# PriviligedLearningDistributedAerial/imitation

Measured on AMD Instinct MI355X. Metric: env-steps/sec (whole node) + final eval return, GAIL HalfCheetah-v4 at 1/2/4/8 MI355X, higher is better.
Workload: dtype mixed (fp32 master weights and accumulation; PPO products as split-bf16 x3 ~fp32, discriminator bf16); 1 GPU; model=GAIL: FeedForward32Policy[32,32]+RunningNorm / BasicRewardNet(32,32)+RunningNorm, global_batch=4096, seq_len=512, parallelism=dp1, engine=device, env=HalfCheetah-v4

## Files before the change

### csrc/kernels/ppo_rc_kernel.h

```cpp
#pragma once
#include <hip/hip_runtime.h>
#include <stdlib.h>

#include "ia/engine.h"
#include "ia/wave.h"
#include "launchers.h"


namespace ia {
namespace rc {


typedef float f4 __attribute__((ext_vector_type(4)));
typedef __bf16 bf16;
typedef __bf16 bf16x8 __attribute__((ext_vector_type(8)));
typedef __attribute__((address_space(3))) bf16 lbf;
typedef __attribute__((address_space(3))) bf16x8 lbf8;
typedef __attribute__((address_space(3))) float lf;
typedef __attribute__((address_space(3))) f4 lf4;

constexpr int kL = kWaveMaxLayers;

__device__ __forceinline__ f4 mfma(float a, float b, f4 c) { return __builtin_amdgcn_mfma_f32_16x16x4f32(a, b, c, 0, 0, 0); }
__device__ __forceinline__ int rfl(int v) { return __builtin_amdgcn_readfirstlane(v); }
// ... 199 lines not shown
}
__device__ __forceinline__ void img_store1(lf* L, int off, int rp, int f, int row, float v) {
  lch* p = (lch*)L + 4 * off + (f >> 4) * img_strip(rp) + img_unit(row, (f >> 2) & 3) + 2 * (f & 3);
  const bf16 h = (bf16)v;
  *(lbf*)p = h;
  *(lbf*)(p + img_lo(rp)) = (bf16)(v - (float)h);
}
__device__ __forceinline__ bf16x8 img_read8(const lch* a0, const lch* a1) {
  const bf16x4 x = __builtin_amdgcn_ds_read_tr16_b64_v4bf16((lbf4*)a0);
  const bf16x4 y = __builtin_amdgcn_ds_read_tr16_b64_v4bf16((lbf4*)a1);
  return cat4(x, y);
}

__device__ __forceinline__ f4 mfma_bf16(bf16x8 a, bf16x8 b, f4 c) { return __builtin_amdgcn_mfma_f32_16x16x32_bf16(a, b, c, 0, 0, 0); }

template <int N>
__device__ __forceinline__ void dw_tiles(const lf* L, const int* izo, const int* iho, int d1, int lo, int ksteps, f4* acc) {
  const lch* Lb = (const lch*)L;
  constexpr int GS = N >= 12 ? 2 : 4;
#pragma unroll
  for (int i0 = 0; i0 < N; i0 += GS) {
    for (int ks = 0; ks < ksteps; ++ks) {
      bf16x8 zh[GS], zl[GS], hh[GS], hl[GS];
#pragma unroll
      for (int i = 0; i < GS; ++i) {
        if (i0 + i >= N) continue;
        const lch* zp = Lb + izo[i0 + i] + kImgKStep * ks;
        const lch* hp = Lb + iho[i0 + i] + kImgKStep * ks;
        zh[i] = img_read8(zp, zp + d1);
        zl[i] = img_read8(zp + lo, zp + lo + d1);
        hh[i] = img_read8(hp, hp + d1);
        hl[i] = img_read8(hp + lo, hp + lo + d1);
      }
#pragma unroll
      for (int i = 0; i < GS; ++i) {
        if (i0 + i >= N) continue;
        acc[i0 + i] = mfma_bf16(zh[i], hh[i], acc[i0 + i]);
        acc[i0 + i] = mfma_bf16(zh[i], hl[i], acc[i0 + i]);
        acc[i0 + i] = mfma_bf16(zl[i], hh[i], acc[i0 + i]);
      }
    }
  }
}

__host__ __device__ __forceinline__ int bf3_ld(int k) { return k + 8; }
__device__ __forceinline__ int bf3_pos_in0(int f) { return 8 * (f & 3) + (f >> 2); }
__device__ __forceinline__ int bf3_pos_h(int f) { return 32 * (f >> 5) + 8 * ((f >> 2) & 3) + 4 * ((f >> 4) & 1) + (f & 3); }

__device__ __forceinline__ void split8(const float (&v)[8], bf16x8& hi, bf16x8& lo) {
#pragma unroll
  for (int j = 0; j < 8; ++j) {
    const bf16 h = (bf16)v[j];
    hi[j] = h;
    lo[j] = (bf16)(v[j] - (float)h);
  }
}

__device__ __forceinline__ f4 bf3_tile(const lbf* a, int lo_off, bf16x8 bh, bf16x8 bl, f4 acc) {
  const bf16x8 ah = *(const lbf8*)a;
  const bf16x8 al = *(const lbf8*)(a + lo_off);
  acc = mfma_bf16(ah, bh, acc);
  acc = mfma_bf16(ah, bl, acc);
  return mfma_bf16(al, bh, acc);
}

__device__ __forceinline__ f4 bf3_mm(bf16x8 ah, bf16x8 al, bf16x8 bh, bf16x8 bl, f4 acc) {
  acc = mfma_bf16(ah, bh, acc);
  acc = mfma_bf16(ah, bl, acc);
  return mfma_bf16(al, bh, acc);
}

template <int KT>
__device__ __forceinline__ void bf3_store_w(lf* L, const PPORcGeo& g, int q, int l, int o, int i, float v, int nl) {
  const bf16 h = (bf16)v;
  const bf16 lo = (bf16)(v - (float)h);
  const int kin = l == 0 ? 32 : 16 * KT;
  const int rows = (g.dout[q][l] + 15) & ~15;
  lbf* wf = (lbf*)(L + g.wf_off[q][l]) + o * bf3_ld(kin) + (l == 0 ? bf3_pos_in0(i) : bf3_pos_h(i));
  wf[0] = h;
  wf[rows * bf3_ld(kin)] = lo;
  if (l > 0) {
    const int kout = l == nl - 1 ? 32 : 16 * KT;
    const int trows = (g.din[q][l] + 15) & ~15;
    lbf* wt = (lbf*)(L + g.wt_off[q][l]) + i * bf3_ld(kout) + bf3_pos_h(o);
    wt[0] = h;
    wt[trows * bf3_ld(kout)] = lo;
  }
}

template <int KT>
__device__ __forceinline__ void bf3_store_tile(lf* L, int kind, int wf, int wfl, int wt, int wtl, int r16, int kk,
                                               const float (&v)[4]) {
  typedef __bf16 bf16x4 __attribute__((ext_vector_type(4)));
  typedef __attribute__((address_space(3))) bf16x4 lbf4;
  bf16x4 h4, l4;
#pragma unroll
  for (int j = 0; j < 4; ++j) {
    const bf16 h = (bf16)v[j];
    h4[j] = h;
    l4[j] = (bf16)(v[j] - (float)h);
  }
  lbf* Lb = (lbf*)L;
  const int ldi = kind == 0 ? bf3_ld(32) : bf3_ld(16 * KT);
  lbf* pf = Lb + wf + 4 * kk * ldi + (kind == 0 ? 8 * (r16 & 3) + (r16 >> 2) : 8 * (r16 >> 2) + (r16 & 3));
#pragma unroll
  for (int j = 0; j < 4; ++j) {
    pf[j * ldi] = h4[j];
    pf[j * ldi + wfl] = l4[j];
  }
  if (kind != 0) {
    const int ldo = kind == 2 ? bf3_ld(32) : bf3_ld(16 * KT);
    lbf* pt = Lb + wt + r16 * ldo + 8 * kk;
    *(lbf4*)pt = h4;
    *(lbf4*)(pt + wtl) = l4;
  }
}

constexpr bool rc_is_bf3(int KT, int S0T, int NLT, int HWT, int CWT, int NW) {
  return HWT == 16 * KT && NLT == 3 && S0T != 0 && (S0T > 0 ? S0T : -S0T) <= 8 && CWT == 64 && (NW == 4 || KT == 2);
}

template <int KT, int KW, int KB, int S0T, int NLT, int ACTT, int HWT, int CWT, int DT, int NW, int LEAN = 0>
__global__ __launch_bounds__(64 * NW) void ppo_rc_kernel(PPOArgs a, PPORcGeo g) {
  constexpr int KI = KW + KB;
  constexpr bool kLean = LEAN != 0;
  unsigned long long* const prof = kLean ? nullptr : a.prof;
  constexpr int kThreads = 64 * NW;
  constexpr int kWaves = NW;
  constexpr int kHalf = NW / 2;
  extern __shared__ __attribute__((aligned(16))) float lds_raw[];
  lf* L = (lf*)lds_raw;
  const int tid = threadIdx.x;
  const int w = rfl(tid >> 6), lane = tid & 63;
  const int r16 = lane & 15, kk = lane >> 4;
  const bool ns = g.ns != 0;
  int bid = (int)blockIdx.x;
  if (g.xcd > 1) {
    if (bid % g.xcd) return;
    bid /= g.xcd;
  }
  const int q = ns ? (bid & 1) : w / kHalf;
  const int gw = ns ? w : w % kHalf;
  const int grp = ns ? (bid >> 1) : bid;
  const int G = kLean ? 1 : g.G, nch = g.nch, cw = CWT > 0 ? CWT : g.cw;
  const int CH = G * nch;
  const int Bg = CH * cw;
  const int RT = cw / 16;
  const bool rows_wave = gw < RT;
  const int nl = NLT > 0 ? NLT : (q == 0 ? a.n_pi : a.n_vf);
  const int D = a.D, A = a.A;
  constexpr int S0M = S0T > 0 ? S0T : (S0T < 0 ? -S0T : 16);
  const int s0 = S0T > 0 ? S0T : (D + 3) / 4;
  constexpr bool BF3 = rc_is_bf3(KT, S0T, NLT, HWT, CWT, NW);
  const bool gauss = DT >= 0 ? DT == 0 : !a.discrete;
  const bool has_ls = gauss && a.log_std_off >= 0;
  float am[4];
#pragma unroll
  for (int j = 0; j < 4; ++j) am[j] = 4 * (lane >> 4) + j < a.A ? 1.f : 0.f;
  const int n_mb = a.rows / Bg;
  const int K = a.n_epochs * n_mb;
  const float invB = 1.f / (float)Bg;
  const float c_half_log2pi = 0.91893853320467274f;
  const int n_items = rfl(g.n_items);

  for (int i = tid; i < g.lds_floats; i += kThreads) L[i] = 0.f;
  __syncthreads();
#pragma unroll
  for (int qq = 0; qq < 2; ++qq) {
#pragma unroll
    for (int l = 0; l < kL; ++l) {
      if (l >= (qq == 0 ? a.n_pi : a.n_vf) || (ns && qq != q)) continue;
      const LG y = lg(g, qq, l);
      const int wo = qq == 0 ? a.pi_w_off[l] : a.vf_w_off[l];
      const int bo = qq == 0 ? a.pi_b_off[l] : a.vf_b_off[l];
      for (int i = tid; i < y.dout * y.din; i += kThreads) {
        const int o = i / y.din, c = i - o * y.din;
        if constexpr (BF3) bf3_store_w<KT>(L, g, qq, l, o, c, a.params[wo + i], qq == 0 ? a.n_pi : a.n_vf);
        else L[y.w + o * y.ldw + c] = a.params[wo + i];
      }
      for (int i = tid; i < y.dout; i += kThreads) L[y.b + i] = a.params[bo + i];
    }
  }
  if (tid < 16) L[g.ls_off + tid] = (has_ls && tid < A && !(ns && q != 0)) ? a.params[a.log_std_off + tid] : 0.f;
  const int nc = tid - (kThreads - 64);
  const bool norm_lane = a.has_norm && nc >= 0 && nc < D;
  float run_m = 0.f, run_v = 1.f, run_c = 0.f;
  if (norm_lane) {
    run_m = a.norm_mean[nc];
    run_v = a.norm_var[nc];
    run_c = a.norm_count_i ? (float)a.norm_count_i[0] : a.norm_count[0];
  }
  const int n_witems = rfl(g.n_witems);
  const int wb = ns ? rfl(g.wbase[q]) : 0, nwq = ns ? rfl(g.nwit[q]) : n_witems;
  const int bb = ns ? rfl(g.bbase[q]) : n_witems, nbq = ns ? rfl(g.nbit[q]) : n_items - n_witems;
  float gm[KW][4], gv[KW][4];
  f4 gg[KW];
  float wmst[BF3 ? KW : 1][4];
  float bm[KB], bv[KB], bg[KB];
#pragma unroll
  for (int it = 0; it < KW; ++it) {
#pragma unroll
    for (int j = 0; j < 4; ++j) gm[it][j] = gv[it][j] = 0.f;
    gg[it] = {0.f, 0.f, 0.f, 0.f};
    if (w + it * kWaves < nwq) {
      const int desc = rfl(g.items[wb + w + it * kWaves]);
      const int iq = desc & 1, il = (desc >> 1) & 3, ta = (desc >> 5) & 15, tb = (desc >> 9) & 15;
      const int din = g.din[iq][il], dout = g.dout[iq][il];
      const int wo = iq == 0 ? a.pi_w_off[il] : a.vf_w_off[il];
      const int in = 16 * tb + r16;
#pragma unroll
      for (int j = 0; j < 4; ++j) {
        const int o = 16 * ta + 4 * kk + j;
        if constexpr (BF3) wmst[it][j] = 0.f;
        if (o < dout && in < din) {
          gm[it][j] = a.exp_avg[wo + o * din + in];
          gv[it][j] = a.exp_avg_sq[wo + o * din + in];
          if constexpr (BF3) wmst[it][j] = a.params[wo + o * din + in];
        }
      }
    }
  }
#pragma unroll
  for (int ib = 0; ib < KB; ++ib) {
    bm[ib] = bv[ib] = bg[ib] = 0.f;
    if (w + ib * kWaves < nbq) {
      const int desc = rfl(g.items[bb + w + ib * kWaves]);
      const int iq = desc & 1, il = (desc >> 1) & 3, kind = (desc >> 3) & 3;
      if (kind == 1) {
        const int dout = g.dout[iq][il];
        const int bo = iq == 0 ? a.pi_b_off[il] : a.vf_b_off[il];
        if (lane < dout) {
          bm[ib] = a.exp_avg[bo + lane];
          bv[ib] = a.exp_avg_sq[bo + lane];
        }
      } else if (has_ls && lane < A) {
        bm[ib] = a.exp_avg[a.log_std_off + lane];
        bv[ib] = a.exp_avg_sq[a.log_std_off + lane];
      }
    }
  }
  float st_ent = 0.f, st_pg = 0.f, st_vl = 0.f, st_cf = 0.f, st_kl = 0.f;
  float step = a.adam_step[0];
  float b1t = powf(a.beta1, step), b2t = powf(a.beta2, step);
  const int hid_act = ACTT >= 0 ? ACTT : a.hidden_act;
  if (norm_lane && K > 0) {
    const float m = g.mom[nc], v = g.mom[64 + nc], n = (float)Bg;
    const float tot = run_c + n, delta = m - run_m;
    run_m += delta * n / tot;
    run_v = (run_v * run_c + v * n + delta * delta * run_c * n / tot) / tot;
    run_c = tot;
    L[g.nm_off + nc] = run_m;
    L[g.nm_off + 64 + nc] = rsqrtf(run_v + a.norm_eps);
  }
  const int nwi = nwq > w ? min(KW, (nwq - w + kWaves - 1) / kWaves) : 0;
  constexpr int rp = CWT > 32 ? CWT : 32;
  constexpr int ksteps = rp / 32;
  int lterm, lterm1;
  img_lane_terms(r16, kk, lterm, lterm1);
  constexpr bool HOIST = NW == 4 && KW <= 8;
  auto slot_dw = [&](int it, int& zu, int& hu) {
    const int desc = rfl(g.items[wb + w + it * kWaves]);
    const int iq = desc & 1, il = (desc >> 1) & 3, ta = (desc >> 5) & 15, tb = (desc >> 9) & 15;
    zu = 4 * rfl(g.z_off[iq][il]) + ta * img_strip(rp);
    hu = 4 * rfl(g.h_off[iq][il]) + tb * img_strip(rp);
  };
  auto slot_img = [&](int it, int& kd, int& wf, int& wl, int& wt, int& tl) {
    const int desc = rfl(g.items[wb + w + it * kWaves]);
    const int iq = desc & 1, il = (desc >> 1) & 3, ta = (desc >> 5) & 15, tb = (desc >> 9) & 15;
    const int nlq = iq == 0 ? a.n_pi : a.n_vf;
    const int ldi = bf3_ld(il == 0 ? 32 : 16 * KT);
    wf = rfl(2 * g.wf_off[iq][il] + 16 * ta * ldi + (il == 0 ? 4 * tb : 32 * (tb >> 1) + 4 * (tb & 1)));
    wl = rfl(((g.dout[iq][il] + 15) & ~15) * ldi);
    kd = il == 0 ? 0 : (il == nlq - 1 ? 2 : 1);
    wt = tl = 0;
    if (il > 0) {
      const int ldo = bf3_ld(il == nlq - 1 ? 32 : 16 * KT);
      wt = rfl(2 * g.wt_off[iq][il] + 16 * tb * ldo + 32 * (ta >> 1) + 4 * (ta & 1));
      tl = rfl(((g.din[iq][il] + 15) & ~15) * ldo);
    }
  };
  constexpr bool GHOIST = HOIST && NLT > 0;
  LG yq[GHOIST ? kL : 1];
  int wfq[GHOIST && BF3 ? kL : 1], wtq[GHOIST && BF3 ? kL : 1];
#pragma unroll
  for (int l = 0; l < kL; ++l) {
    if (!GHOIST || l >= nl) continue;
    yq[GHOIST ? l : 0] = lg(g, q, l);
    if constexpr (BF3) {
      wfq[GHOIST ? l : 0] = rfl(g.wf_off[q][l]);
      wtq[GHOIST ? l : 0] = rfl(g.wt_off[q][l]);
    }
  }
  auto LY = [&](int l) -> LG {
    if constexpr (GHOIST) return yq[GHOIST ? l : 0];
    else return lg(g, q, l);
  };
  auto WF = [&](int l) -> int {
    if constexpr (GHOIST && BF3) return wfq[GHOIST ? l : 0];
    else return rfl(g.wf_off[q][l]);
  };
  auto WT = [&](int l) -> int {
    if constexpr (GHOIST && BF3) return wtq[GHOIST ? l : 0];
    else return rfl(g.wt_off[q][l]);
  };
  constexpr int KH = HOIST ? KW : 1, KHB = HOIST && BF3 ? KW : 1;
  int izu[KH], ihu[KH];
  int bwf[KHB], bwt[KHB], bpk[KHB];
#pragma unroll
  for (int it = 0; it < KH; ++it) {
    izu[it] = ihu[it] = 0;
    if (HOIST && it < nwi) slot_dw(it, izu[it], ihu[it]);
  }
#pragma unroll
  for (int it = 0; it < KHB; ++it) {
    bwf[it] = bwt[it] = bpk[it] = 0;
    if (HOIST && BF3 && it < nwi) {
      int kd, wl, tl;
      slot_img(it, kd, bwf[it], wl, bwt[it], tl);
      bpk[it] = kd | (wl << 2) | (tl << 17);
    }
  }
  int bkind[KB], b_off[KB], b_addr[KB];
  float b_okf[KB];
#pragma unroll
  for (int ib = 0; ib < KB; ++ib) {
    bkind[ib] = -1;
    b_off[ib] = 0;
    b_okf[ib] = 0.f;
    b_addr[ib] = g.trash_off + lane;
    if (w + ib * kWaves >= nbq) continue;
    const int desc = rfl(g.items[bb + w + ib * kWaves]);
    const int iq = desc & 1, il = (desc >> 1) & 3, kind = (desc >> 3) & 3;
    const LG y = lg(g, iq, il);
    bkind[ib] = kind;
    b_off[ib] = kind == 1 ? y.db : g.lsp_off;
    const bool ok = kind == 1 ? (lane < y.dout) : (has_ls && lane < A);
    b_okf[ib] = ok ? 1.f : 0.f;
    if (ok) b_addr[ib] = kind == 1 ? y.b + lane : g.ls_off + lane;
  }
  float pre_m = 0.f, pre_v = 0.f;
  if (norm_lane && K > 1) {
    pre_m = g.mom[128 + nc];
    pre_v = g.mom[128 + 64 + nc];
  }
  Rows<S0M> cur;
  const int row = 16 * gw + r16;
  const int sterm = img_unit(row, kk);
  auto slot_of = [&](int u) -> size_t { return (size_t)(u / nch) * CH + (size_t)grp * nch + (u % nch); };
  if (rows_wave && K > 0) load_rows(g, slot_of(0), row, kk, s0, cur);
  __shared__ unsigned long long sprof[20];
  if (tid < 20) sprof[tid] = 0;
  unsigned* arrive = g.sync + (ns ? 4 * q : 0);
  unsigned* tflag = g.sync + 1;
  unsigned* arrive2 = g.sync + (ns ? 4 * q + 2 : 2);
  const unsigned spin_lim = a.spin_limit ? a.spin_limit : (1u << 22);
  const bool stall = a.debug_stall != 0 && bid == (ns ? 2 * G : G) - 1;
  __syncthreads();

  auto norm_rows = [&](int nbuf, float (&xo)[S0M]) {
    float nmv[S0M], nrv[S0M];
#pragma unroll
    for (int s = 0; s < S0M; ++s) {
      nmv[s] = 0.f;
      nrv[s] = 1.f;
      if (s < s0 && a.has_norm) {
        nmv[s] = L[g.nm_off + nbuf + 4 * s + kk];
        nrv[s] = L[g.nm_off + nbuf + 64 + 4 * s + kk];
      }
    }
#pragma unroll
    for (int s = 0; s < S0M; ++s) xo[s] = s < s0 ? (cur.x[s] - nmv[s]) * nrv[s] : 0.f;
    if (q == 0 || ns) {
      const int h0 = rfl(g.h_off[0][0]);
#pragma unroll
      for (int s = 0; s < S0M; ++s)
        if (s < s0) img_store1(L, h0, rp, 4 * s + kk, row, xo[s]);
    }
  };
  constexpr bool PREC = KW <= 8;
  const bool pre = PREC && (ns || G > 1) && (kLean || g.xstash < 0);
  float xpre[PREC ? S0M : 1];
#pragma unroll
  for (int s = 0; s < (PREC ? S0M : 1); ++s) xpre[s] = 0.f;
  auto pre_rows = [&](int k) {
    if constexpr (PREC)
      if (pre && rows_wave && k + 1 < K) norm_rows(((k + 1) & 1) * 128, xpre);
  };

  constexpr bool kEarly = KW <= 8;
  float step_size = 0.f, inv_bc2s = 0.f;
  auto adam_scalars = [&]() {
    step += 1.f;
    b1t *= a.beta1;
    b2t *= a.beta2;
    step_size = a.lr / (1.f - b1t);
    inv_bc2s = 1.f / sqrtf(1.f - b2t);
  };

  constexpr bool PREF = BF3 && KT == 2 && NW == 4;
  constexpr int PL = PREF ? NLT : 1, PT = PREF ? KT : 1;
  bf16x8 pwf[PL][PT][2], pwt[PL][PT][2];
  f4 pbs[PL][PT];
  f4 pls = {0.f, 0.f, 0.f, 0.f};

  for (int k = 0; k < K; ++k) {
    unsigned long long t0 = prof ? clock64() : 0;
    const int nb = (k & 1) * 128;
    if constexpr (PREF) {
      if (rows_wave) {
        pls = *(const lf4*)(L + g.ls_off + 4 * kk);
#pragma unroll
        for (int l = 0; l < PL; ++l) {
          const LG y = LY(l);
          const bool last = l == PL - 1;
          const int kin = l == 0 ? 32 : 16 * KT;
          const int rows = (y.dout + 15) & ~15;
          const lbf* wf = (const lbf*)(L + WF(l)) + r16 * bf3_ld(kin) + 8 * kk;
#pragma unroll
          for (int t = 0; t < PT; ++t) {
            if (last && t > 0) continue;
            pwf[l][t][0] = *(const lbf8*)(wf + 16 * t * bf3_ld(kin));
            pwf[l][t][1] = *(const lbf8*)(wf + 16 * t * bf3_ld(kin) + rows * bf3_ld(kin));
            pbs[l][t] = *(const lf4*)(L + y.b + 16 * t + 4 * kk);
          }
          if (l == 0) continue;
          const int kout = last ? 32 : 16 * KT;
          const int trows = (y.din + 15) & ~15;
          const lbf* wt_img = (const lbf*)(L + WT(l)) + r16 * bf3_ld(kout) + 8 * kk;
#pragma unroll
          for (int u2 = 0; u2 < PT; ++u2) {
            pwt[l][u2][0] = *(const lbf8*)(wt_img + 16 * u2 * bf3_ld(kout));
            pwt[l][u2][1] = *(const lbf8*)(wt_img + 16 * u2 * bf3_ld(kout) + trows * bf3_ld(kout));
          }
        }
      }
    }
#pragma unroll
    for (int it = 0; it < KW; ++it) gg[it] = {0.f, 0.f, 0.f, 0.f};
#pragma unroll
    for (int ib = 0; ib < KB; ++ib) bg[ib] = 0.f;
    for (int ch = 0; ch < nch; ++ch) {
      const int u = k * nch + ch;
      Rows<S0M> nxt;
      if (rows_wave && u + 1 < K * nch) load_rows(g, slot_of(u + 1), row, kk, s0, nxt);
      float mom_m = 0.f, mom_v = 0.f;
      if (ch == 0 && norm_lane) {
        mom_m = pre_m;
        mom_v = pre_v;
        if (k + 2 < K) {
          pre_m = g.mom[(size_t)(k + 2) * 128 + nc];
          pre_v = g.mom[(size_t)(k + 2) * 128 + 64 + nc];
        }
      }
      unsigned long long c0 = prof ? clock64() : 0;
      if (rows_wave) {
        float xb[S0M];
        if constexpr (PREC) {
          if (pre && ch == 0 && k > 0) {
#pragma unroll
            for (int s = 0; s < S0M; ++s) xb[s] = xpre[s];
          } else {
            norm_rows(nb, xb);
          }
        } else {
          float nmv[S0M], nrv[S0M];
#pragma unroll
          for (int s = 0; s < S0M; ++s) {
            nmv[s] = 0.f;
            nrv[s] = 1.f;
            if (s < s0 && a.has_norm) {
              nmv[s] = L[g.nm_off + nb + 4 * s + kk];
              nrv[s] = L[g.nm_off + nb + 64 + 4 * s + kk];
            }
          }
#pragma unroll
          for (int s = 0; s < S0M; ++s) xb[s] = s < s0 ? (cur.x[s] - nmv[s]) * nrv[s] : 0.f;
          if (q == 0 || ns) {
            const int h0 = rfl(g.h_off[0][0]);
#pragma unroll
            for (int s = 0; s < S0M; ++s)
              if (s < s0) img_store1(L, h0, rp, 4 * s + kk, row, xb[s]);
          }
        }
        unsigned long long c1 = prof ? clock64() : 0;
        f4 hreg[kL - 1][KT];
        bf16x4 hsp[kL - 1][KT][2];
        f4 head = {0.f, 0.f, 0.f, 0.f};
#pragma unroll
        for (int l = 0; l < kL; ++l) {
          if (l >= nl) continue;
          const LG y = LY(l);
          const bool last = l == nl - 1;
          const int tout = last ? 1 : (HWT > 0 ? HWT / 16 : ((y.dout + 15) >> 4));
          f4 acc[KT];
#pragma unroll
          for (int t = 0; t < KT; ++t) acc[t] = {0.f, 0.f, 0.f, 0.f};
          if constexpr (BF3) {
            constexpr int KS = KT / 2;
            const int ks_l = l == 0 ? 1 : KS;
            const int kin = l == 0 ? 32 : 16 * KT;
            const int rows = (y.dout + 15) & ~15;
            const lbf* wf = (const lbf*)(L + WF(l)) + r16 * bf3_ld(kin) + 8 * kk;
#pragma unroll
            for (int ks = 0; ks < KS; ++ks) {
              if (ks >= ks_l) continue;
              bf16x8 bh, bl;
              if (l == 0) {
                float v[8];
#pragma unroll
                for (int j = 0; j < 8; ++j) v[j] = j < S0M ? xb[j < S0M ? j : 0] : 0.f;
                split8(v, bh, bl);
              } else {
                bh = cat4(hsp[l > 0 ? l - 1 : 0][2 * ks][0], hsp[l > 0 ? l - 1 : 0][2 * ks + 1][0]);
                bl = cat4(hsp[l > 0 ? l - 1 : 0][2 * ks][1], hsp[l > 0 ? l - 1 : 0][2 * ks + 1][1]);
              }
#pragma unroll
              for (int t = 0; t < KT; ++t) {
                if (t >= tout) continue;
                if constexpr (PREF) acc[t] = bf3_mm(pwf[PREF ? l : 0][PREF ? t : 0][0], pwf[PREF ? l : 0][PREF ? t : 0][1], bh, bl, acc[t]);
                else acc[t] = bf3_tile(wf + 16 * t * bf3_ld(kin) + 32 * ks, rows * bf3_ld(kin), bh, bl, acc[t]);
              }
            }
          } else if (l == 0 && KT > 2) {
#pragma unroll
            for (int t0 = 0; t0 < KT; t0 += 2) {
              float w0[2][S0M];
#pragma unroll
              for (int t = 0; t < 2; ++t)
#pragma unroll
                for (int s = 0; s < S0M; ++s)
                  if (t0 + t < tout && s < s0) w0[t][s] = L[y.w + (16 * (t0 + t) + r16) * y.ldw + 4 * s + kk];
#pragma unroll
              for (int s = 0; s < S0M; ++s)
#pragma unroll
                for (int t = 0; t < 2; ++t)
                  if (t0 + t < tout && s < s0) acc[t0 + t] = mfma(w0[t][s], xb[s], acc[t0 + t]);
            }
          } else if (l == 0) {
            float w0[KT][S0M];
#pragma unroll
            for (int t = 0; t < KT; ++t)
#pragma unroll
              for (int s = 0; s < S0M; ++s)
                if (t < tout && s < s0) w0[t][s] = L[y.w + (16 * t + r16) * y.ldw + 4 * s + kk];
#pragma unroll
            for (int s = 0; s < S0M; ++s)
#pragma unroll
              for (int t = 0; t < KT; ++t)
                if (t < tout && s < s0) acc[t] = mfma(w0[t][s], xb[s], acc[t]);
          } else if constexpr (KT > 2) {
            const int tin = HWT > 0 ? HWT / 16 : ((y.din + 15) >> 4);
#pragma unroll
            for (int t = 0; t < KT; ++t) {
              if (t >= tout) continue;
              const lf* wr = L + y.w + (16 * t + r16) * y.ldw;
#pragma unroll
              for (int h = 0; h < KT; ++h) {
                if (h >= tin) continue;
                const f4 w4 = *(const lf4*)(wr + 16 * h + 4 * kk);
                acc[t] = mfma(w4.x, hreg[l - 1][h].x, acc[t]);
                acc[t] = mfma(w4.y, hreg[l - 1][h].y, acc[t]);
                acc[t] = mfma(w4.z, hreg[l - 1][h].z, acc[t]);
                acc[t] = mfma(w4.w, hreg[l - 1][h].w, acc[t]);
              }
            }
          } else {
            const int tin = HWT > 0 ? HWT / 16 : ((y.din + 15) >> 4);
            f4 w4[KT][KT];
#pragma unroll
            for (int t = 0; t < KT; ++t)
#pragma unroll
              for (int h = 0; h < KT; ++h)
                if (t < tout && h < tin) w4[t][h] = *(const lf4*)(L + y.w + (16 * t + r16) * y.ldw + 16 * h + 4 * kk);
#pragma unroll
            for (int h = 0; h < KT; ++h) {
#pragma unroll
              for (int t = 0; t < KT; ++t) {
                if (t >= tout || h >= tin) continue;
                acc[t] = mfma(w4[t][h].x, hreg[l - 1][h].x, acc[t]);
                acc[t] = mfma(w4[t][h].y, hreg[l - 1][h].y, acc[t]);
                acc[t] = mfma(w4[t][h].z, hreg[l - 1][h].z, acc[t]);
                acc[t] = mfma(w4[t][h].w, hreg[l - 1][h].w, acc[t]);
              }
            }
          }
#pragma unroll
          for (int t = 0; t < KT; ++t) {
            if (t >= tout) continue;
            const int o0 = 16 * t + 4 * kk;
            f4 bb;
            if constexpr (PREF) bb = pbs[PREF ? l : 0][PREF ? t : 0];
            else bb = *(const lf4*)(L + y.b + o0);
            f4 v;
            v.x = acc[t].x + bb.x;
            v.y = acc[t].y + bb.y;
            v.z = acc[t].z + bb.z;
            v.w = acc[t].w + bb.w;
            if (!last) {
              v.x = (HWT > 0 || o0 + 0 < y.dout) ? act_fn(hid_act, v.x) : 0.f;
              v.y = (HWT > 0 || o0 + 1 < y.dout) ? act_fn(hid_act, v.y) : 0.f;
              v.z = (HWT > 0 || o0 + 2 < y.dout) ? act_fn(hid_act, v.z) : 0.f;
              v.w = (HWT > 0 || o0 + 3 < y.dout) ? act_fn(hid_act, v.w) : 0.f;
              if (l < kL - 1) {
                hreg[l][t] = v;
// ... 61 lines not shown
          const float lr_ = logp - old_lp;
          const float ratio = expf(lr_);
          const float lo = 1.f - a.clip_range, hi = 1.f + a.clip_range;
          const float pl1 = adv * ratio, pl2 = adv * fminf(fmaxf(ratio, lo), hi);
          float c1, c2;
          if (pl1 < pl2) { c1 = 1.f; c2 = 0.f; } else if (pl2 < pl1) { c1 = 0.f; c2 = 1.f; } else { c1 = 0.5f; c2 = 0.5f; }
          const float inside = (ratio >= lo && ratio <= hi) ? 1.f : 0.f;
          const float dlogp = -invB * (c1 * adv + c2 * adv * inside) * ratio;
          if (gauss) {
            float lsp[4];
#pragma unroll
            for (int j = 0; j < 4; ++j) {
              const int o = 4 * kk + j;
              dzv[j] = dlogp * zs[j] * isd[j];
              lsp[j] = am[j] * dlogp * (zs[j] * zs[j] - 1.f);
            }
#pragma unroll
            for (int j = 0; j < 4; ++j) {
              const float s = sum16(lsp[j]);
              if (r16 == 0) L[g.lsp_off + gw * 16 + 4 * kk + j] = s;
            }
          } else {
#pragma unroll
            for (int j = 0; j < 4; ++j) {
              const int o = 4 * kk + j;
              dzv[j] = o < yh.dout ? dlogp * ((o == act_row ? 1.f : 0.f) - pk[j]) -
                                         a.ent_coef * invB * (-pk[j] * (lpk[j] + ent_row))
                                   : 0.f;
            }
          }
          dz = {dzv[0], dzv[1], dzv[2], dzv[3]};
          if (kk == 0) {
            st_pg += -fminf(pl1, pl2);
            st_cf += fabsf(ratio - 1.f) > a.clip_range ? 1.f : 0.f;
            st_kl += (ratio - 1.f) - lr_;
            if (!gauss) st_ent += -ent_row;
          }
        } else {
          float d = 0.f;
          if (kk == 0) {
            d = head.x - cur.rd.z;
            st_vl += d * d;
          }
          dz = {kk == 0 ? a.vf_coef * 2.f * d * invB : 0.f, 0.f, 0.f, 0.f};
        }
        unsigned long long c3 = prof ? clock64() : 0;
        f4 dzc[KT];
        dzc[0] = dz;
#pragma unroll
        for (int t = 1; t < KT; ++t) dzc[t] = {0.f, 0.f, 0.f, 0.f};
#pragma unroll
        for (int l = kL - 1; l >= 0; --l) {
          if (l >= nl) continue;
          const LG y = LY(l);
          const int tout = l == nl - 1 ? 1 : (HWT > 0 ? HWT / 16 : ((y.dout + 15) >> 4));
          const int tin = HWT > 0 ? HWT / 16 : ((y.din + 15) >> 4);
          constexpr int KWT = KT > 2 ? 1 : KT;
          float wt[KWT][KWT][4];
          if (!BF3 && KT <= 2 && l > 0) {
#pragma unroll
            for (int u2 = 0; u2 < KT; ++u2)
#pragma unroll
              for (int tt = 0; tt < KT; ++tt)
#pragma unroll
                for (int j = 0; j < 4; ++j)
                  if (u2 < tin && tt < tout) wt[u2 % KWT][tt % KWT][j] = L[y.w + (16 * tt + 4 * kk + j) * y.ldw + 16 * u2 + r16];
          }
          bf16x4 zsp[KT][2];
#pragma unroll
          for (int u2 = 0; u2 < KT; ++u2) zsp[u2][0] = zsp[u2][1] = bf16x4{(bf16)0.f, (bf16)0.f, (bf16)0.f, (bf16)0.f};
#pragma unroll
          for (int u2 = 0; u2 < KT; ++u2) {
            if (u2 >= tout) continue;
            split4(dzc[u2], zsp[u2][0], zsp[u2][1]);
            img_store4(L, y.z, rp, u2, sterm, zsp[u2][0], zsp[u2][1]);
            const float s0v = sum16(dzc[u2].x), s1v = sum16(dzc[u2].y), s2v = sum16(dzc[u2].z), s3v = sum16(dzc[u2].w);
            if (r16 == 0) {
              const f4 sv = {s0v, s1v, s2v, s3v};
              *(lf4*)(L + y.db + gw * 64 + 16 * u2 + 4 * kk) = sv;
            }
          }
          if (l == 0) break;
          f4 accb[KT];
#pragma unroll
          for (int u2 = 0; u2 < KT; ++u2) accb[u2] = {0.f, 0.f, 0.f, 0.f};
          if constexpr (BF3) {
            constexpr int KS = KT / 2;
            const bool head = l == nl - 1;
            const int ks_l = head ? 1 : KS;
            const int kout = head ? 32 : 16 * KT;
            const int trows = (y.din + 15) & ~15;
            const lbf* wt_img = (const lbf*)(L + WT(l)) + r16 * bf3_ld(kout) + 8 * kk;
#pragma unroll
            for (int ks = 0; ks < KS; ++ks) {
              if (ks >= ks_l) continue;
              const bf16x8 bh = cat4(zsp[2 * ks][0], zsp[2 * ks + 1][0]), bl = cat4(zsp[2 * ks][1], zsp[2 * ks + 1][1]);
#pragma unroll
              for (int u2 = 0; u2 < KT; ++u2) {
                if (u2 >= tin) continue;
                if constexpr (PREF) accb[u2] = bf3_mm(pwt[PREF ? l : 0][PREF ? u2 : 0][0], pwt[PREF ? l : 0][PREF ? u2 : 0][1], bh, bl, accb[u2]);
                else accb[u2] = bf3_tile(wt_img + 16 * u2 * bf3_ld(kout) + 32 * ks, trows * bf3_ld(kout), bh, bl, accb[u2]);
              }
            }
          } else if constexpr (KT <= 2) {
#pragma unroll
            for (int tt = 0; tt < KT; ++tt)
#pragma unroll
              for (int j = 0; j < 4; ++j)
#pragma unroll
                for (int u2 = 0; u2 < KT; ++u2)
                  if (u2 < tin && tt < tout) accb[u2] = mfma(wt[u2 % KWT][tt % KWT][j], dzc[tt][j], accb[u2]);
          } else {
#pragma unroll
            for (int u2 = 0; u2 < KT; ++u2) {
              if (u2 >= tin) continue;
#pragma unroll
              for (int tt = 0; tt < KT; ++tt) {
                if (tt >= tout) continue;
                const lf* wc = L + y.w + (16 * tt + 4 * kk) * y.ldw + 16 * u2 + r16;
                accb[u2] = mfma(wc[0], dzc[tt].x, accb[u2]);
                accb[u2] = mfma(wc[y.ldw], dzc[tt].y, accb[u2]);
                accb[u2] = mfma(wc[2 * y.ldw], dzc[tt].z, accb[u2]);
                accb[u2] = mfma(wc[3 * y.ldw], dzc[tt].w, accb[u2]);
              }
            }
          }
          f4 nd[KT];
#pragma unroll
          for (int u2 = 0; u2 < KT; ++u2) {
            nd[u2] = {0.f, 0.f, 0.f, 0.f};
            if (u2 >= tin) continue;
            const f4 acc = accb[u2];
            const f4 hv = hreg[l > 0 ? l - 1 : 0][u2];
            nd[u2].x = acc.x * act_grad(hid_act, hv.x);
            nd[u2].y = acc.y * act_grad(hid_act, hv.y);
            nd[u2].z = acc.z * act_grad(hid_act, hv.z);
            nd[u2].w = acc.w * act_grad(hid_act, hv.w);
          }
#pragma unroll
          for (int u2 = 0; u2 < KT; ++u2) dzc[u2] = nd[u2];
        }
        if (prof && lane == 0 && gw == 0) {
          const unsigned long long c4 = clock64();
          const int pb = q == 1 ? 7 : 3;
          sprof[pb + 0] += c1 - c0;
          sprof[pb + 1] += c2 - c1;
          sprof[pb + 2] += c3 - c2;
          sprof[pb + 3] += c4 - c3;
        }
      }
      const unsigned long long cb0 = prof ? clock64() : 0;
      __syncthreads();
      const unsigned long long cb1 = prof ? clock64() : 0;
      if (ch == 0 && norm_lane && k + 1 < K) {
        const float n = (float)Bg;
        const float tot = run_c + n, delta = mom_m - run_m;
        run_m += delta * n / tot;
        run_v = (run_v * run_c + mom_v * n + delta * delta * run_c * n / tot) / tot;
        run_c = tot;
        L[g.nm_off + (128 - nb) + nc] = run_m;
        L[g.nm_off + (128 - nb) + 64 + nc] = rsqrtf(run_v + a.norm_eps);
      }

      {
        int izo[KW], iho[KW];
#pragma unroll
        for (int it = 0; it < KW; ++it) {
          izo[it] = iho[it] = 4 * rfl(g.h_off[0][0]) + lterm;
          if (it < nwi) {
            int zu, hu;
            if constexpr (HOIST) {
              zu = izu[it];
              hu = ihu[it];
            } else {
              slot_dw(it, zu, hu);
            }
            izo[it] = zu + lterm;
            iho[it] = hu + lterm;
          }
        }
        dw_tiles<KW>(L, izo, iho, lterm1 - lterm, img_lo(rp), ksteps, gg);
      }
#pragma unroll
      for (int ib = 0; ib < KB; ++ib) {
        if (bkind[ib] <= 0) continue;
        {
          const int stride = bkind[ib] == 1 ? 64 : 16;
          float gval = 0.f;
          for (int r = 0; r < RT; ++r) gval += L[b_off[ib] + r * stride + lane];
          bg[ib] += gval * b_okf[ib];
        }
      }
      if (prof && tid == 0) {
        sprof[11] += cb1 - cb0;
        sprof[12] += clock64() - cb1;
      }
      if (rows_wave) cur = nxt;
      if (ch + 1 < nch) __syncthreads();
    }
    unsigned long long t1 = prof ? clock64() : 0;

    if constexpr (!kLean) if (G > 1) {
      int ids[KI];
      f4 xg[KI];
#pragma unroll
      for (int it = 0; it < KW; ++it) {
        ids[it] = it < nwi ? wb + w + it * kWaves : -1;
        xg[it] = gg[it];
      }
#pragma unroll
      for (int ib = 0; ib < KB; ++ib) {
        ids[KW + ib] = bkind[ib] >= 0 ? bb + w + ib * kWaves : -1;
        xg[KW + ib] = {bg[ib], 0.f, 0.f, 0.f};
      }
      float* slab = g.slab + (size_t)(k & 1) * G * n_items * 256;
#pragma unroll
      for (int it = 0; it < KI; ++it) {
        if (ids[it] < 0) continue;
        st_sc1_x4(slab + ((size_t)grp * n_items + ids[it]) * 256 + lane * 4, xg[it]);
      }
      const unsigned long long e0 = prof ? clock64() : 0;
      asm volatile("s_waitcnt vmcnt(0)" ::: "memory");
      __syncthreads();
      const unsigned long long e1 = prof ? clock64() : 0;
      if (tid == 0 && !stall) atomicAdd(arrive, 1u);
      pre_rows(k);
      if (tid == 0) {
        const unsigned target = (unsigned)G * (unsigned)(k + 1);
        unsigned spins = 0;
        while (ld_sc1u(arrive) < target) {
          __builtin_amdgcn_s_sleep(1);
          if (++spins > spin_lim || ld_sc1u(tflag) != 0u) {
            spin_give_up(a, tflag);
            break;
          }
        }
      }
      __syncthreads();
      const unsigned long long e2 = prof ? clock64() : 0;
      if (g.xchg2) {
        float* red = g.red + (size_t)(k & 1) * n_items * 256;
        const size_t gs = (size_t)n_items * 256;
        const auto slot_id = [&](int sl) -> int {
          if (sl < KW) return sl < nwi ? wb + w + sl * kWaves : -1;
          return w + (sl - KW) * kWaves < nbq ? bb + w + (sl - KW) * kWaves : -1;
        };
        if (G == 2) reduce_slots<2, KI>(slab, red, gs, grp, lane, slot_id);
        else if (G == 4) reduce_slots<4, KI>(slab, red, gs, grp, lane, slot_id);
        else if (G == 8) reduce_slots<8, KI>(slab, red, gs, grp, lane, slot_id);
        else if (G == 16) reduce_slots<16, KI>(slab, red, gs, grp, lane, slot_id);
        else if (g.xstash >= 0) {
          lf* st = L + g.xstash;
          const int m = nwq + nbq;
          for (int j = grp; j < m; j += G) {
            const int id = j < nwq ? wb + j : bb + (j - nwq);
            const float* p = slab + (size_t)id * 256 + lane * 4;
            f4 v[16];
#pragma unroll
            for (int e = 0; e < 16; ++e) {
              const int gi = w + e * kWaves;
              v[e] = {0.f, 0.f, 0.f, 0.f};
              if (gi < G) v[e] = ld_sc1_x4(p + (size_t)gi * gs);
            }
            wait_vm_n<16>(v);
#pragma unroll
            for (int e = 0; e < 16; ++e) {
              const int gi = w + e * kWaves;
              if (gi < G) *(lf4*)(st + gi * 256 + lane * 4) = v[e];
            }
            __syncthreads();
            for (int el = tid; el < 256; el += kThreads) {
              float sacc = st[el];
#pragma unroll 8
              for (int gi = 1; gi < G; ++gi) sacc += st[gi * 256 + el];
              st_sc1_x1(red + (size_t)id * 256 + el, sacc);
            }
            __syncthreads();
          }
          if (grp < m)
            for (int i = tid; i < G * 64; i += kThreads) *(lf4*)(st + 4 * i) = f4{0.f, 0.f, 0.f, 0.f};
        } else {
#pragma unroll
          for (int it = 0; it < KI; ++it) {
            const int id = ids[it];
            if (id < 0 || it % G != grp) continue;
            const float* p = slab + (size_t)id * 256 + lane * 4;
            f4 sacc = {0.f, 0.f, 0.f, 0.f};
            for (int gi0 = 0; gi0 < G; gi0 += 16) {
              f4 v[16];
#pragma unroll
              for (int e = 0; e < 16; ++e) v[e] = ld_sc1_x4(p + (size_t)(gi0 + e < G ? gi0 + e : 0) * gs);
              wait_vm_n<16>(v);
              if (gi0 == 0) sacc = v[0];
              else sacc += v[0];
#pragma unroll
              for (int e = 1; e < 16; ++e)
                if (gi0 + e < G) sacc += v[e];
            }
            st_sc1_x4(red + (size_t)id * 256 + lane * 4, sacc);
          }
        }
        asm volatile("s_waitcnt vmcnt(0)" ::: "memory");
        __syncthreads();
        if (tid == 0) {
          if (!stall) atomicAdd(arrive2, 1u);
          const unsigned target = (unsigned)G * (unsigned)(k + 1);
          unsigned spins = 0;
          while (ld_sc1u(arrive2) < target) {
            __builtin_amdgcn_s_sleep(1);
            if (++spins > spin_lim || ld_sc1u(tflag) != 0u) {
              spin_give_up(a, tflag);
              break;
            }
          }
        }
        __syncthreads();
#pragma unroll
        for (int it = 0; it < KI; ++it) xg[it] = ld_sc1_x4(red + (size_t)(ids[it] >= 0 ? ids[it] : 0) * 256 + lane * 4);
        wait_vm_n<KI>(xg);
      } else if (G == 2) {
        exchange_sum<2, KI>(slab, n_items, ids, lane, xg);
      } else if (G == 4) {
        exchange_sum<4, KI>(slab, n_items, ids, lane, xg);
      } else if (G == 8) {
        exchange_sum<8, KI>(slab, n_items, ids, lane, xg);
      } else {
#pragma unroll
        for (int it = 0; it < KI; ++it) {
          if (ids[it] < 0) continue;
          f4 sacc = {0.f, 0.f, 0.f, 0.f};
          const float* p = slab + (size_t)ids[it] * 256 + lane * 4;
          const size_t gs = (size_t)n_items * 256;
          for (int gi = 0; gi < G; gi += 4) {
            f4 v0 = ld_sc1_x4(p + (size_t)gi * gs);
            f4 v1 = ld_sc1_x4(p + (size_t)(gi + 1 < G ? gi + 1 : 0) * gs);
            f4 v2 = ld_sc1_x4(p + (size_t)(gi + 2 < G ? gi + 2 : 0) * gs);
            f4 v3 = ld_sc1_x4(p + (size_t)(gi + 3 < G ? gi + 3 : 0) * gs);
            wait_vm4(v0, v1, v2, v3);
            sacc += v0;
            if (gi + 1 < G) sacc += v1;
            if (gi + 2 < G) sacc += v2;
            if (gi + 3 < G) sacc += v3;
          }
          xg[it] = sacc;
        }
      }
#pragma unroll
      for (int it = 0; it < KW; ++it) {
        if (ids[it] < 0) continue;
        gg[it] = xg[it];
      }
#pragma unroll
      for (int ib = 0; ib < KB; ++ib)
        if (ids[KW + ib] >= 0) bg[ib] = xg[KW + ib].x;
      if (prof && tid == 0) {
        sprof[13] += e1 - e0;
        sprof[14] += e2 - e1;
        sprof[15] += clock64() - e2;
      }
    }
    float ss = 0.f;
#pragma unroll
    for (int it = 0; it < KW; ++it) {
      if (it >= nwi) continue;
#pragma unroll
      for (int j = 0; j < 4; ++j) ss += gg[it][j] * gg[it][j];
    }
#pragma unroll
    for (int ib = 0; ib < KB; ++ib) {
      if (bkind[ib] < 0) continue;
      if (bkind[ib] == 2) bg[ib] -= a.ent_coef * b_okf[ib];
      ss += bg[ib] * bg[ib];
    }
    ss = wave_sum(ss);
    if (lane == 0) L[g.red_off + w] = ss;
    if (gauss && tid == 0 && grp == 0 && q == 0) {
      float sl = 0.f;
      for (int j = 0; j < A; ++j) sl += has_ls ? L[g.ls_off + j] : 0.f;
      st_ent += -(sl + A * (0.5f + c_half_log2pi));
    }
    if (kEarly && !ns) adam_scalars();
    __syncthreads();
    unsigned long long t2 = prof ? clock64() : 0;

    float tot = 0.f;
#pragma unroll
    for (int i = 0; i < kWaves; ++i) tot += L[g.red_off + i];
    if (ns) {
      const unsigned long long x0 = prof ? clock64() : 0;
      unsigned long long* xs = reinterpret_cast<unsigned long long*>(g.sync + 8);
      const unsigned long long tag = (unsigned long long)(unsigned)(k + 1) << 32;
      if (tid == 0 && !stall) __hip_atomic_store(xs + q, tag | __float_as_uint(tot), __ATOMIC_RELAXED, __HIP_MEMORY_SCOPE_AGENT);
      unsigned long long o = 0;
      if (kEarly && tid == 0) o = __hip_atomic_load(xs + (1 - q), __ATOMIC_RELAXED, __HIP_MEMORY_SCOPE_AGENT);
      if (G == 1) pre_rows(k);
      if (kEarly) adam_scalars();
      if (tid == 0) {
        if (!kEarly) o = __hip_atomic_load(xs + (1 - q), __ATOMIC_RELAXED, __HIP_MEMORY_SCOPE_AGENT);
        unsigned spins = 0;
        while ((o >> 32) != (unsigned long long)(unsigned)(k + 1)) {
          __builtin_amdgcn_s_sleep(1);
          if (++spins > spin_lim || ld_sc1u(tflag) != 0u) {
            spin_give_up(a, tflag);
            break;
          }
          o = __hip_atomic_load(xs + (1 - q), __ATOMIC_RELAXED, __HIP_MEMORY_SCOPE_AGENT);
        }
        const float other = __uint_as_float((unsigned)(o & 0xffffffffu));
        L[g.red_off + 48] = q == 0 ? tot + other : other + tot;
      }
      __syncthreads();
      tot = L[g.red_off + 48];
      if (prof && tid == 0) sprof[16] += clock64() - x0;
    }
    constexpr bool kProfAdam = KW <= 8;
    if (kProfAdam && prof && tid == 0) sprof[17] -= clock64();
    if (!kEarly) adam_scalars();
    const float coef = fminf(1.f, a.max_grad_norm / (sqrtf(tot) + 1e-6f));
    const float b1 = a.beta1, b2 = a.beta2, eps = a.adam_eps;
    int paddr[KW];
    int pstr[KW];
#pragma unroll
    for (int it = 0; it < KW; ++it) {
      paddr[it] = g.trash_off + lane;
      pstr[it] = 0;
      if (it < nwi) {
        const int desc = rfl(g.items[wb + w + it * kWaves]);
        const int iq = desc & 1, il = (desc >> 1) & 3, ta = (desc >> 5) & 15, tb = (desc >> 9) & 15;
        const int ldw = rfl(g.ldw[iq][il]);
        paddr[it] = rfl(g.w_off[iq][il]) + (16 * ta + 4 * kk) * ldw + 16 * tb + r16;
        pstr[it] = ldw;
      }
    }
    float pval[KW][4], bval[KB];
#pragma unroll
    for (int it = 0; it < KW; ++it)
#pragma unroll
      for (int j = 0; j < 4; ++j) {
        if constexpr (BF3) pval[it][j] = wmst[it][j];
        else pval[it][j] = L[paddr[it] + j * pstr[it]];
      }
#pragma unroll
    for (int ib = 0; ib < KB; ++ib) bval[ib] = L[b_addr[ib]];
#pragma unroll
    for (int it = 0; it < KW; ++it) {
      if (it >= nwi) continue;
#pragma unroll
      for (int j = 0; j < 4; ++j) {
        const float gval = gg[it][j] * coef;
        gm[it][j] = b1 * gm[it][j] + (1.f - b1) * gval;
        gv[it][j] = b2 * gv[it][j] + (1.f - b2) * gval * gval;
        const float denom = __builtin_amdgcn_sqrtf(gv[it][j]) * inv_bc2s + eps;
        const float nv = pval[it][j] - step_size * gm[it][j] * __builtin_amdgcn_rcpf(denom);
        if constexpr (BF3) wmst[it][j] = nv;
        else L[paddr[it] + j * pstr[it]] = nv;
      }
      if constexpr (BF3) {
        if constexpr (HOIST) {
          bf3_store_tile<KT>(L, bpk[it] & 3, bwf[it], (bpk[it] >> 2) & 0x7fff, bwt[it], bpk[it] >> 17, r16, kk, wmst[it]);
        } else {
          int kd, wf, wl, wt, tl;
          slot_img(it, kd, wf, wl, wt, tl);
          bf3_store_tile<KT>(L, kd, wf, wl, wt, tl, r16, kk, wmst[it]);
        }
      }
    }
#pragma unroll
    for (int ib = 0; ib < KB; ++ib) {
      if (bkind[ib] < 0) continue;
      const float gval = bg[ib] * coef;
      bm[ib] = b1 * bm[ib] + (1.f - b1) * gval;
      bv[ib] = b2 * bv[ib] + (1.f - b2) * gval * gval;
      const float denom = __builtin_amdgcn_sqrtf(bv[ib]) * inv_bc2s + eps;
      L[b_addr[ib]] = bval[ib] - step_size * bm[ib] * __builtin_amdgcn_rcpf(denom);
    }
    if (kProfAdam && prof && tid == 0) {
      const unsigned long long a1 = clock64();
      sprof[17] += a1;
      sprof[18] -= a1;
    }
    __syncthreads();
    if (prof && tid == 0) {
      const unsigned long long t3 = clock64();
      sprof[0] += t1 - t0;
      sprof[1] += t2 - t1;
      sprof[2] += t3 - t2;
      if (kProfAdam) sprof[18] += t3;
    }
  }

  const float vals[5] = {st_ent, st_pg, st_vl, st_cf, st_kl};
#pragma unroll
  for (int i = 0; i < 5; ++i) {
    const float v = wave_sum(vals[i]);
    if (lane == 0) L[g.red_off + 8 + w * 5 + i] = v;
  }
  __syncthreads();
  if (tid < 5) {
    float s = 0.f;
    for (int i = 0; i < kWaves; ++i) s += L[g.red_off + 8 + i * 5 + tid];
    if (!(tid == 0 && gauss)) s *= invB;
    if (G > 1 || ns) atomicAdd(a.stats + tid, s);
    else a.stats[tid] += s;
  }
  if (grp != 0) return;
  const bool shared_wb = !ns || q == 0;

#pragma unroll
  for (int qq = 0; qq < 2; ++qq) {
#pragma unroll
    for (int l = 0; l < kL; ++l) {
      if (l >= (qq == 0 ? a.n_pi : a.n_vf) || (ns && qq != q)) continue;
      const LG y = lg(g, qq, l);
      const int wo = qq == 0 ? a.pi_w_off[l] : a.vf_w_off[l];
      const int bo = qq == 0 ? a.pi_b_off[l] : a.vf_b_off[l];
      if constexpr (!BF3)
        for (int i = tid; i < y.dout * y.din; i += kThreads) {
          const int o = i / y.din, c = i - o * y.din;
          a.params[wo + i] = L[y.w + o * y.ldw + c];
        }
      for (int i = tid; i < y.dout; i += kThreads) a.params[bo + i] = L[y.b + i];
    }
  }
  if (shared_wb && has_ls && tid < A) a.params[a.log_std_off + tid] = L[g.ls_off + tid];
#pragma unroll
  for (int it = 0; it < KW; ++it) {
    if (it >= nwi) continue;
    const int desc = rfl(g.items[wb + w + it * kWaves]);
    const int iq = desc & 1, il = (desc >> 1) & 3, ta = (desc >> 5) & 15, tb = (desc >> 9) & 15;
    const int din = g.din[iq][il], dout = g.dout[iq][il];
    const int wo = iq == 0 ? a.pi_w_off[il] : a.vf_w_off[il];
    const int in = 16 * tb + r16;
#pragma unroll
    for (int j = 0; j < 4; ++j) {
      const int o = 16 * ta + 4 * kk + j;
      if (o < dout && in < din) {
        a.exp_avg[wo + o * din + in] = gm[it][j];
        a.exp_avg_sq[wo + o * din + in] = gv[it][j];
        if constexpr (BF3) a.params[wo + o * din + in] = wmst[it][j];
      }
    }
  }
#pragma unroll
  for (int ib = 0; ib < KB; ++ib) {
    if (bkind[ib] < 0 || b_okf[ib] == 0.f) continue;
    const int desc = rfl(g.items[bb + w + ib * kWaves]);
    const int iq = desc & 1, il = (desc >> 1) & 3;
    const int off = bkind[ib] == 1 ? (iq == 0 ? a.pi_b_off[il] : a.vf_b_off[il]) : a.log_std_off;
    a.exp_avg[off + lane] = bm[ib];
    a.exp_avg_sq[off + lane] = bv[ib];
  }
  if (shared_wb && norm_lane && K > 0) {
    a.norm_mean[nc] = run_m;
    a.norm_var[nc] = run_v;
    if (nc == 0) {
      if (a.norm_count_i) a.norm_count_i[0] = (int)run_c;
      else a.norm_count[0] = run_c;
    }
  }
  if (shared_wb && tid == 0) a.adam_step[0] = step;
  if (prof && tid < 20) {
    const bool critic_slot = tid >= 7 && tid <= 10;
    if (!ns) prof[tid] += sprof[tid];
    else if (q == 0 && !critic_slot) prof[tid] += sprof[tid];
    else if (q == 1 && critic_slot) atomicAdd(prof + tid, sprof[tid]);
  }
}

}
}
```

Baseline: 1.704 million env-steps/s.

## Move running-norm merge and entropy sum off the chunk critical path

For the KB==1, NW==4 specialization, the running observation-norm merge for minibatch k+2 now runs after the Adam update in the last wave, using a double-buffered norm table. Before, it ran inside the chunk loop right after a barrier. The entropy log-std sum moves from a serial tid==0 loop after the reduction into a vectorized LDS read done by one wave. The bias-gradient row sum is unrolled with loads issued before the adds. When S0T is fixed and there is no norm, the norm table is pre-filled with identity values so norm_rows can read it without branching. The intent is to shorten the serial work between barriers, at the cost of more complex prefetch indexing, where an off-by-one in the k+2/k+3 schedule could corrupt the normalization.

Result: faster. 1.934 million env-steps/s (median of 6 runs) (+13.5%).

```diff
diff --git a/csrc/kernels/ppo_rc_kernel.h b/csrc/kernels/ppo_rc_kernel.h
--- a/csrc/kernels/ppo_rc_kernel.h
+++ b/csrc/kernels/ppo_rc_kernel.h
@@ -375,6 +375,8 @@
   constexpr int S0M = S0T > 0 ? S0T : (S0T < 0 ? -S0T : 16);
   const int s0 = S0T > 0 ? S0T : (D + 3) / 4;
   constexpr bool BF3 = rc_is_bf3(KT, S0T, NLT, HWT, CWT, NW);
+  constexpr bool kOffPath = KB == 1 && NW == 4;
+  constexpr bool kNormBatch = kOffPath && S0T > 0 && KW <= 8;
   const bool gauss = DT >= 0 ? DT == 0 : !a.discrete;
   const bool has_ls = gauss && a.log_std_off >= 0;
   float am[4];
@@ -405,6 +407,8 @@
     }
   }
   if (tid < 16) L[g.ls_off + tid] = (has_ls && tid < A && !(ns && q != 0)) ? a.params[a.log_std_off + tid] : 0.f;
+  if constexpr (kNormBatch)
+    if (!a.has_norm && tid < 64) L[g.nm_off + 64 + tid] = L[g.nm_off + 128 + 64 + tid] = 1.f;
   const int nc = tid - (kThreads - 64);
   const bool norm_lane = a.has_norm && nc >= 0 && nc < D;
   float run_m = 0.f, run_v = 1.f, run_c = 0.f;
@@ -466,15 +470,17 @@
   float step = a.adam_step[0];
   float b1t = powf(a.beta1, step), b2t = powf(a.beta2, step);
   const int hid_act = ACTT >= 0 ? ACTT : a.hidden_act;
-  if (norm_lane && K > 0) {
-    const float m = g.mom[nc], v = g.mom[64 + nc], n = (float)Bg;
-    const float tot = run_c + n, delta = m - run_m;
+  auto norm_merge = [&](float mom_m, float mom_v, int half) {
+    const float n = (float)Bg;
+    const float tot = run_c + n, delta = mom_m - run_m;
     run_m += delta * n / tot;
-    run_v = (run_v * run_c + v * n + delta * delta * run_c * n / tot) / tot;
+    run_v = (run_v * run_c + mom_v * n + delta * delta * run_c * n / tot) / tot;
     run_c = tot;
-    L[g.nm_off + nc] = run_m;
-    L[g.nm_off + 64 + nc] = rsqrtf(run_v + a.norm_eps);
-  }
+    L[g.nm_off + half + nc] = run_m;
+    L[g.nm_off + half + 64 + nc] = rsqrtf(run_v + a.norm_eps);
+  };
+  if (norm_lane && K > 0) norm_merge(g.mom[nc], g.mom[64 + nc], 0);
+  if (kOffPath && norm_lane && K > 1) norm_merge(g.mom[128 + nc], g.mom[128 + 64 + nc], 128);
   const int nwi = nwq > w ? min(KW, (nwq - w + kWaves - 1) / kWaves) : 0;
   constexpr int rp = CWT > 32 ? CWT : 32;
   constexpr int ksteps = rp / 32;
@@ -562,9 +568,10 @@
     if (ok) b_addr[ib] = kind == 1 ? y.b + lane : g.ls_off + lane;
   }
   float pre_m = 0.f, pre_v = 0.f;
-  if (norm_lane && K > 1) {
-    pre_m = g.mom[128 + nc];
-    pre_v = g.mom[128 + 64 + nc];
+  constexpr int kAhead = kOffPath ? 2 : 1;
+  if (norm_lane && K > kAhead) {
+    pre_m = g.mom[kAhead * 128 + nc];
+    pre_v = g.mom[kAhead * 128 + 64 + nc];
   }
   Rows<S0M> cur;
   const int row = 16 * gw + r16;
@@ -584,11 +591,16 @@
     float nmv[S0M], nrv[S0M];
 #pragma unroll
     for (int s = 0; s < S0M; ++s) {
-      nmv[s] = 0.f;
-      nrv[s] = 1.f;
-      if (s < s0 && a.has_norm) {
+      if constexpr (kNormBatch) {
         nmv[s] = L[g.nm_off + nbuf + 4 * s + kk];
         nrv[s] = L[g.nm_off + nbuf + 64 + 4 * s + kk];
+      } else {
+        nmv[s] = 0.f;
+        nrv[s] = 1.f;
+        if (s < s0 && a.has_norm) {
+          nmv[s] = L[g.nm_off + nbuf + 4 * s + kk];
+          nrv[s] = L[g.nm_off + nbuf + 64 + 4 * s + kk];
+        }
       }
     }
 #pragma unroll
@@ -626,6 +638,9 @@
   f4 pbs[PL][PT];
   f4 pls = {0.f, 0.f, 0.f, 0.f};
 
+  const bool ent_wave = kOffPath && gauss && grp == 0 && (!ns || q == 0) && w == kWaves - 1;
+  float ent_sl = 0.f;
+
   for (int k = 0; k < K; ++k) {
     unsigned long long t0 = prof ? clock64() : 0;
     const int nb = (k & 1) * 128;
@@ -667,12 +682,14 @@
       Rows<S0M> nxt;
       if (rows_wave && u + 1 < K * nch) load_rows(g, slot_of(u + 1), row, kk, s0, nxt);
       float mom_m = 0.f, mom_v = 0.f;
-      if (ch == 0 && norm_lane) {
-        mom_m = pre_m;
-        mom_v = pre_v;
-        if (k + 2 < K) {
-          pre_m = g.mom[(size_t)(k + 2) * 128 + nc];
-          pre_v = g.mom[(size_t)(k + 2) * 128 + 64 + nc];
+      if constexpr (!kOffPath) {
+        if (ch == 0 && norm_lane) {
+          mom_m = pre_m;
+          mom_v = pre_v;
+          if (k + 2 < K) {
+            pre_m = g.mom[(size_t)(k + 2) * 128 + nc];
+            pre_v = g.mom[(size_t)(k + 2) * 128 + 64 + nc];
+          }
         }
       }
       unsigned long long c0 = prof ? clock64() : 0;
@@ -1040,14 +1057,18 @@
       const unsigned long long cb0 = prof ? clock64() : 0;
       __syncthreads();
       const unsigned long long cb1 = prof ? clock64() : 0;
-      if (ch == 0 && norm_lane && k + 1 < K) {
-        const float n = (float)Bg;
-        const float tot = run_c + n, delta = mom_m - run_m;
-        run_m += delta * n / tot;
-        run_v = (run_v * run_c + mom_v * n + delta * delta * run_c * n / tot) / tot;
-        run_c = tot;
-        L[g.nm_off + (128 - nb) + nc] = run_m;
-        L[g.nm_off + (128 - nb) + 64 + nc] = rsqrtf(run_v + a.norm_eps);
+      if constexpr (!kOffPath)
+        if (ch == 0 && norm_lane && k + 1 < K) norm_merge(mom_m, mom_v, 128 - nb);
+      if (ent_wave) {
+        f4 e4[4];
+#pragma unroll
+        for (int i = 0; i < 4; ++i) e4[i] = *(const lf4*)(L + g.ls_off + 4 * i);
+        float sl = 0.f;
+#pragma unroll
+        for (int i = 0; i < 4; ++i)
+#pragma unroll
+          for (int j = 0; j < 4; ++j) sl += e4[i][j];
+        ent_sl = sl;
       }
 
       {
@@ -1075,7 +1096,16 @@
         {
           const int stride = bkind[ib] == 1 ? 64 : 16;
           float gval = 0.f;
-          for (int r = 0; r < RT; ++r) gval += L[b_off[ib] + r * stride + lane];
+          if constexpr (kOffPath && CWT > 0) {
+            constexpr int RTC = CWT / 16;
+            float pv[RTC];
+#pragma unroll
+            for (int r = 0; r < RTC; ++r) pv[r] = L[b_off[ib] + r * stride + lane];
+#pragma unroll
+            for (int r = 0; r < RTC; ++r) gval += pv[r];
+          } else {
+            for (int r = 0; r < RT; ++r) gval += L[b_off[ib] + r * stride + lane];
+          }
           bg[ib] += gval * b_okf[ib];
         }
       }
@@ -1262,7 +1292,12 @@
     }
     ss = wave_sum(ss);
     if (lane == 0) L[g.red_off + w] = ss;
-    if (gauss && tid == 0 && grp == 0 && q == 0) {
+    if constexpr (kOffPath) {
+      if (ent_wave && lane == 0) {
+        const float sl = ent_sl;
+        st_ent += -(sl + A * (0.5f + c_half_log2pi));
+      }
+    } else if (gauss && tid == 0 && grp == 0 && q == 0) {
       float sl = 0.f;
       for (int j = 0; j < A; ++j) sl += has_ls ? L[g.ls_off + j] : 0.f;
       st_ent += -(sl + A * (0.5f + c_half_log2pi));
@@ -1362,6 +1397,15 @@
       const float denom = __builtin_amdgcn_sqrtf(bv[ib]) * inv_bc2s + eps;
       L[b_addr[ib]] = bval[ib] - step_size * bm[ib] * __builtin_amdgcn_rcpf(denom);
     }
+    if (kOffPath && w == kWaves - 1 && k + 2 < K) {
+      if (norm_lane) {
+        norm_merge(pre_m, pre_v, nb);
+        if (k + 3 < K) {
+          pre_m = g.mom[(size_t)(k + 3) * 128 + nc];
+          pre_v = g.mom[(size_t)(k + 3) * 128 + 64 + nc];
+        }
+      }
+    }
     if (kProfAdam && prof && tid == 0) {
       const unsigned long long a1 = clock64();
       sprof[17] += a1;
```
